# kai0511/insider

Hardware: AMD Instinct MI355X
Metric: outer-iterations/sec (masked INSIDER fit, 10000 x 50000, K=30) (higher is better)
Workload: dtype f64

## Files before the change

### insider_amd/csrc/insider_hip.hip

```cpp
#include "insider_kernels.hpp"
#include "insider_posthoc.hpp"
#include "insider_vardecomp.hpp"
#include "insider_sampdecomp.hpp"
#include "insider_levelscores.hpp"
#include "insider_factdecomp.hpp"
#include "insider_rescomp.hpp"
#include "insider_outliers.hpp"
#include "insider_neighbors.hpp"
#include "insider_coexpr.hpp"
#include "insider_coexpr_pc.hpp"
#include "insider_enrich.hpp"
#include "insider_kmeans.hpp"
#include "insider_hclust.hpp"
#include "insider_tsne.hpp"

#include <rccl/rccl.h>

#include <algorithm>
#include <chrono>
#include <cstdlib>
#include <cmath>
#include <cstdio>
#include <cstring>
#include <limits>
// ... 214 lines not shown
    std::vector<CovTables> contm;
    CovTables contm_lists;
    DevBuf<double> cont_cnt;
    bool cont_merged = false;
    std::vector<DevBuf<double>> cont_pair;
    std::shared_ptr<const HostTables> host;
    mutable std::mutex fold_mu;
    mutable std::shared_ptr<const FoldIds> folds;
    std::shared_ptr<const FoldIds> get_folds() const { std::lock_guard<std::mutex> g(fold_mu); return folds; }
    size_t bytes_shared = 0, bytes_own = 0;

    struct Block { int rows, off; };
    int blocks() const { return c + (m > 0 ? 1 : 0); }
    Block block(int b) const { return b < c ? Block{n_levels[b], lvl_off[b]} : Block{m, SLcat}; }

    DataSet() = default;
    DataSet(const DataSet &) = delete;
    DataSet &operator=(const DataSet &) = delete;
    ~DataSet() { (void)hipSetDevice(device); }
};

struct Workspace {
    static constexpr int EARLY = 3;
    int K = 0, NB = 0, KP = 0, nseg = 1;
    int gram_blocks_p = 0, gram_blocks_n = 0, sc_blocks = 0;
    DevBuf<double> Astack, R, C, RtR, CCt, Qfull, SC, stat, stat_col, gram_part, sc_part, lvl_part, eq, lvl_sum;
    DevBuf<double> fperm;
    DevBuf<double> lvl_zero;
    DevBuf<double> Qheld;
    DevBuf<double> U, Ylvl, wpart, Vlev;
    DevBuf<double> lvl_sum_all;
    DevBuf<double> gram_part2, sc_part2;
    DevBuf<double> wg_part;
    DevBuf<uint8_t> wg_pair;
    DevBuf<double> sse_train, sse_test, b2, b1, loss_buf, stage;
    size_t stage_count = 0;
    DevBuf<int> sweeps, failflag;
    DevBuf<int> sweep_key;
    DevBuf<unsigned long long> sweep_total;
    DevBuf<unsigned> pc4_ticket;
    unsigned pc4_base[2] = {0, 0};
    unsigned long long cd_code_base = 0, cd_pair_base = 0;
    DevBuf<unsigned long long> code_base_dev;
    uint8_t *order = nullptr;
    DevBuf<uint8_t> order_buf[2];
    int order_rows = 0;
    DevBuf<int> gene_perm;
    DevBuf<int> sched_cnt[2], sched_rank;
    DevBuf<uint16_t> sched_bkt;
    int sched_flip = 0;
    DevBuf<double> cd_hsave, cd_isave;
    DevBuf<uint32_t> cd_pass_slot;
    DevBuf<int> cd_pass_perm[2], cd_pass_cnt;
    DevBuf<int> perm_early[EARLY];
    bool have_early[EARLY] = {false, false, false};
    bool have_perm = false;
};

constexpr unsigned EV_SYNC = hipEventDisableTiming | hipEventDisableSystemFence;

struct Join {
    Event ev;
    bool pending = false;
    int record(hipStream_t s) { HIPCHECK(hipEventRecord(ev, s)); pending = true; return INSIDER_OK; }
    int wait(hipStream_t s)
    {
        if (pending) HIPCHECK(hipStreamWaitEvent(s, ev, 0));
        pending = false;
        return INSIDER_OK;
    }
    void drop() { pending = false; }
};

struct Streams {
    Stream stream;
    Stream side;
    Stream side2;
    Stream side3;
    Event ev_cd_done, ev_prep, ev_c_ready;
    Event ev_head;
    std::vector<Event> ev_w;
    Event ev_a_ready, ev_tab;
    Join qfull, qheld, side_done;

    int create(int n_w)
    {
        HIPCHECK(hipStreamCreate(stream.out()));
        for (Stream *s : {&side, &side2, &side3}) HIPCHECK(hipStreamCreateWithFlags(s->out(), hipStreamNonBlocking));
        for (Event *e : {&ev_prep, &ev_c_ready, &ev_head, &ev_a_ready, &qfull.ev, &qheld.ev, &ev_cd_done, &side_done.ev, &ev_tab})
            HIPCHECK(hipEventCreateWithFlags(e->out(), EV_SYNC));
        ev_w.resize(n_w);
        for (Event &e : ev_w) HIPCHECK(hipEventCreateWithFlags(e.out(), EV_SYNC));
        return INSIDER_OK;
    }
    int synchronize_sides() const
    {
        for (const Stream *s : {&side, &side2, &side3}) HIPCHECK(hipStreamSynchronize(*s));
        return INSIDER_OK;
    }
    void synchronize() const
    {
        for (const Stream *s : {&stream, &side, &side2, &side3}) if (*s) (void)hipStreamSynchronize(*s);
    }
};

struct Options {
    int max_sweeps = 1 << 24, order_mode = 0, profile = 0, verbose = 0, cd_variant = 0, force_allreduce = 0;
    int col_factored = 1;
    int row_counts = 1;
    int row_merged = 1;
    int row_gemm = 1;
    int wg_waves = 1024;
    int row_fused = 1;
    int mm_fast = 1;
    int mm_tiles = 0;
    int col_mfma4 = 1;
    int stats_own_q = 1;
    int cd_pairs = 1;
    int list_fine = 1;
    int cd_cold_iters = 3, cd_pass_first = 64, cd_pass_ratio = 4;
    double resid_stage_mb = 256.0;
    double vd_stage_kb = 48.0;
    int sd_slabs = 0;
    int ls_slabs = 0;
    double ls_part_mb = 256.0;
    int glm_slabs = 0;
    int rc_slabs = 0;
};

struct PostWs {
    DevBuf<double> Ast, U, cp, part, stats, stage, gpart, gram, cpart, gsum, L, dinv, outs;
    DevBuf<int> nz, ints, info;
    DevBuf<double> vin, vtab, vrec;
    DevBuf<double> spart, srec;
    DevBuf<double> lcand, ltab, lpart, lcnt, lout;
    DevBuf<double> fwall, fprod, fbase, frec;
    DevBuf<double> rq, rcs, rz, rpart, rin, rout;
    DevBuf<double> ocs, oz;
    DevBuf<uint32_t> obits;
    DevBuf<int> ogcnt, oscnt, orows, ocols;
    DevBuf<long long> ooffs;
};

}

struct insider_hip_handle {
    std::shared_ptr<const DataSet> ds;
    Streams st;
    Options opt;
    Workspace ws;
    PostWs post;
    FitPlan plan;
    bool w_ready = false;
    int64_t gene_offset = 0;
    int rank = 0, world = 1;
    insider_allreduce_fn allreduce = nullptr;
    void *allreduce_user = nullptr;
    ncclComm_t comm = nullptr;
    std::vector<Event> ev_col, ev_row, ev_cd, ev_test;
    double prof[12] = {0, 0, 0, 0, 0, 0, 0, 0, 0, 0, 0, 0};
    double steady_cd_ms = 0, steady_col_ms = 0;
    int cap_hits = 0, max_gene_sweeps = 0;
    int col_solver = 0, col_eval = 0, col_ridge_fallback = 0;
    int col_stats_kernel = 0, col_stats_tickets = 0, col_stats_blocks = 0;
    int col_stats_own_q = 0;
    int col_q_kernel = 0, mm_rows2_tiles = 0;
    uint64_t row_kernels = 0;
    int vd_path = 0;
    int sd_path = 0, sd_slabs = 0;
    int ls_path = 0, ls_slabs = 0;
    int glm_slabs = 0, glm_form = 0;
    int fd_path = 0;
    int ls_form = 0, fd_form = 0, rc_form = 0, cx_form = 0;
    int rc_slabs = 0;
    double rc_ms = 0.0;
    double cx_stage_mb = 0.0, cx_stage_ms = 0.0, cx_ms = 0.0, cx_pc_ms = 0.0;
    int ol_path = 0;

    ~insider_hip_handle()
    {
        if (ds) (void)hipSetDevice(ds->device);
        st.synchronize();
        if (comm) (void)ncclCommDestroy(comm);
    }
};

namespace {

enum RowKernel {
    RK_WGEMM4 = 0, RK_WGEMM5, RK_WGEMM6, RK_WGEMM7, RK_WGEMM_CHUNKS, RK_WSYRK, RK_GRAM_SIDE,
    RK_GENE_U_CNT, RK_GENE_U, RK_GENE_UC,
    RK_MERGED_SOLVE, RK_MERGED, RK_MERGED_ZERO, RK_PACK_REDUCE,
    RK_LIST_STATS4, RK_LIST_STATS, RK_LEVEL_PARTIAL, RK_LEVEL_SOLVE, RK_CONT_CD,
    RK_MM_ROWS2, RK_MM_ROWS, RK_MM_REDUCE2_2, RK_MM_REDUCE2_4, RK_MM_REDUCE
};
inline uint64_t rk_bit(RowKernel k) { return 1ull << (int)k; }
inline void row_mark(insider_hip_handle *h, RowKernel k) { h->row_kernels |= rk_bit(k); }

PlanFacts plan_facts(const insider_hip_handle *h, int K)
{
    const DataSet &d = *h->ds;
    PlanFacts f;
    const Options &o = h->opt;
    f.opt = {o.row_merged, o.col_factored, o.row_fused, o.row_gemm, o.row_counts, o.mm_fast, o.force_allreduce, o.wg_waves,
             o.list_fine, o.mm_tiles, o.col_mfma4, o.cd_variant, o.cd_pairs, o.cd_cold_iters, o.cd_pass_first, o.cd_pass_ratio, o.max_sweeps,
             o.stats_own_q};
    f.world = h->world; f.n_simd = d.n_simd;
    f.K = K; f.NB = h->ws.NB; f.KP = h->ws.KP; f.lvl_zero = (bool)h->ws.lvl_zero; f.fperm = (bool)h->ws.fperm;
    f.merged = d.merged; f.cont_merged = d.cont_merged; f.cf_pair_ok = d.cf_pair_ok; f.cf_hn = (bool)d.cf_hn; f.cf_zt = (bool)d.cf_zt; f.cf_sq = (bool)d.cf_sq;
    f.c = d.c; f.m = d.m; f.SL = d.SL; f.SLP = d.SLP; f.SLcat = d.SLcat; f.n = d.n; f.p = d.p; f.col_entries = d.col_entries; f.row_entries = d.row_entries;
    for (const CovTables &ct : d.cov) { f.L.push_back(ct.L); f.npairs.push_back(ct.npairs); }
    f.cf_c = d.cf.c; f.cf_tab_rows = d.cf.tab_rows; f.cf_nsteps = d.cf.nsteps;
    std::copy(d.cf.L, d.cf.L + CF_MAXC + 1, f.cf_L);
    std::copy(d.cf.nlater, d.cf.nlater + CF_MAXC + 1, f.cf_nlater);
    return f;
}

int ensure_workspace(insider_hip_handle *h, int K)
{
    if (K < 1 || K > INSIDER_MAX_K) return fail(INSIDER_ERR_UNSUPPORTED, "K must be in 1..63");
    if (h->ws.K == K) return INSIDER_OK;
    h->ws = Workspace();
    const DataSet &d = *h->ds;
    const hipStream_t st = h->st.stream;
    Workspace w;
    const int NB = (K + 1 + 15) / 16, KP = 16 * NB, NBLK = NB * (NB + 1) / 2, STAT = NBLK * 256;
    w.NB = NB;
    w.KP = KP;
    const int64_t avg_batches = (int64_t)(d.row_entries / (uint64_t)LIST_ALIGN / (uint64_t)std::max<int64_t>(d.n, 1));
    int nseg = (int)std::min<int64_t>(std::max<int64_t>(1, cdiv(8192, d.n)), std::max<int64_t>(1, avg_batches / 16));
    nseg = std::min(nseg, 64);
    w.nseg = nseg;
    w.gram_blocks_p = cdiv(d.p, MM_SLAB);
    w.gram_blocks_n = cdiv(d.n, MM_SLAB);
    w.sc_blocks = cdiv(d.p, MM_SLAB);
    const size_t rec = STAT + 2 * KP + 2, max_L = std::max(d.max_L, 1);
    int rc;
    if ((rc = w.Astack.alloc((size_t)(d.SL + 16) * KP))) return rc;
    HIPCHECK(hipMemset(w.Astack, 0, (size_t)(d.SL + 16) * KP * sizeof(double)));
    if ((rc = w.R.alloc((size_t)d.n * KP))) return rc;
    if ((rc = w.C.alloc((size_t)(std::max<int64_t>(d.p, d.ldp) + 4) * KP))) return rc;
    if ((rc = w.RtR.alloc((size_t)KP * KP))) return rc;
    if ((rc = w.CCt.alloc((size_t)KP * KP))) return rc;
    if ((rc = w.Qfull.alloc((size_t)d.p * KP))) return rc;
    if ((rc = w.SC.alloc((size_t)d.SL * KP))) return rc;
    if ((rc = w.stat.alloc((size_t)nseg * d.n * STAT))) return rc;
    if ((rc = w.stat_col.alloc((size_t)d.p * STAT))) return rc;
    if ((rc = w.gram_part.alloc((size_t)std::max(w.gram_blocks_p, w.gram_blocks_n) * KP * KP))) return rc;
    if ((rc = w.sc_part.alloc((size_t)w.sc_blocks * d.SL * KP))) return rc;
    if ((rc = w.lvl_part.alloc((size_t)d.max_chunks * rec))) return rc;
    if ((rc = w.lvl_sum.alloc(max_L * rec))) return rc;
    if (NB == 2 && K >= 16)
        if ((rc = w.fperm.alloc((size_t)std::max(d.n, d.p) * KP))) return rc;
    if ((rc = w.lvl_zero.alloc(max_L * rec))) return rc;
    HIPCHECK(hipMemsetAsync(w.lvl_zero, 0, max_L * rec * sizeof(double), st));
    if (d.merged) {
        size_t wg_len = 0;
        int wg_ntile = 0;
        const PlanFacts facts = plan_facts(h, K);
        for (int i = 0; i < d.c; ++i) {
            const WgPlan g = wgemm_plan(facts, i, true);
            if (g.use) {
                wg_len = std::max(wg_len, (size_t)g.nslab * (16 * g.tiles) * (16 * g.ntile));
                wg_ntile = g.ntile;
            }
        }
        if (wg_len) {
            if ((rc = w.wg_part.alloc(wg_len))) return rc;
            std::vector<uint8_t> ab((size_t)2 * 16 * wg_ntile, (uint8_t)(KP - 1));
            int idx = 0;
            for (int a = 0; a < K; ++a)
                for (int b = 0; b <= a; ++b, ++idx) {
                    ab[idx] = (uint8_t)a;
                    ab[(size_t)16 * wg_ntile + idx] = (uint8_t)b;
                }
            if ((rc = w.wg_pair.upload(ab))) return rc;
        }
        if ((rc = w.U.alloc((size_t)d.p * round_up(max_L, 2)))) return rc;
        if ((rc = w.Ylvl.alloc(max_L * KP))) return rc;
        if ((rc = w.wpart.alloc((size_t)std::max(d.max_items, 1) * STAT))) return rc;
        if ((rc = w.lvl_sum_all.alloc((size_t)std::max(d.SL, 1) * rec))) return rc;
        if ((rc = w.gram_part2.alloc((size_t)std::max(w.gram_blocks_p, w.gram_blocks_n) * KP * KP))) return rc;
        if ((rc = w.sc_part2.alloc((size_t)w.sc_blocks * d.SL * KP))) return rc;
        if ((rc = w.Vlev.alloc((size_t)d.p * d.SLP))) return rc;
        HIPCHECK(hipMemsetAsync(w.Vlev, 0, (size_t)d.p * d.SLP * sizeof(double), st));
        if ((rc = w.Qheld.alloc((size_t)d.p * KP))) return rc;
    }
    if ((rc = w.eq.alloc((size_t)d.max_L * (KP * KP + KP)))) return rc;
    for (DevBuf<double> *b : {&w.sse_train, &w.sse_test, &w.b2, &w.b1})
        if ((rc = b->alloc((size_t)d.p))) return rc;
    if ((rc = w.loss_buf.alloc(8))) return rc;
    w.stage_count = (size_t)std::max<int64_t>(std::max<int64_t>(d.p, d.n), d.SL) * KP;
    if ((rc = w.stage.alloc(w.stage_count))) return rc;
    if ((rc = w.sweeps.alloc((size_t)d.p))) return rc;
    if ((rc = w.failflag.alloc(4))) return rc;
    if ((rc = w.sweep_total.alloc(256))) return rc;
    if ((rc = w.pc4_ticket.alloc((size_t)(PC4_PARTS + 1) * 32))) return rc;
    HIPCHECK(hipMemsetAsync(w.pc4_ticket, 0, (size_t)(PC4_PARTS + 1) * 32 * sizeof(unsigned), st));
    if ((rc = w.gene_perm.alloc((size_t)d.p))) return rc;
    if ((rc = w.sched_cnt[0].alloc((size_t)SCHED_BUCKETS))) return rc;
    if ((rc = w.sched_cnt[1].alloc((size_t)SCHED_BUCKETS))) return rc;
    if ((rc = w.sched_rank.alloc((size_t)d.p))) return rc;
    if ((rc = w.sched_bkt.alloc((size_t)d.p))) return rc;
    if ((rc = w.sweep_key.alloc((size_t)d.p))) return rc;
    if ((rc = w.cd_hsave.alloc((size_t)d.p * KP))) return rc;
    if ((rc = w.cd_isave.alloc((size_t)d.p * KP))) return rc;
// ... 586 lines not shown
            HIPCHECK(hipStreamWaitEvent(h->st.side, h->st.ev_cd_done, 0));
            st = h->st.side;
        }
        if ((rc = launch_gene_order(h, h->ws.sweeps, (outer_iter < Workspace::EARLY || !h->ws.have_perm) ? 1 : 0, 0, st, fused_bucket)))
            return rc;
        h->ws.have_perm = true;
        if (early) {
            HIPCHECK(hipMemcpyAsync(h->ws.perm_early[outer_iter], h->ws.gene_perm, (size_t)h->ds->p * sizeof(int),
                                    hipMemcpyDeviceToDevice, st));
            h->ws.have_early[outer_iter] = true;
        }
        if (side) h->st.side_done.pending = true;
    }
    return INSIDER_OK;
}

int side_close(insider_hip_handle *h)
{
    return h->st.side_done.pending ? h->st.side_done.record(h->st.side) : INSIDER_OK;
}

int launch_test_sse(insider_hip_handle *h, int masked, bool timed)
{
    if (!masked) {
        HIPCHECK(hipMemsetAsync(h->ws.sse_test, 0, (size_t)h->ds->p * sizeof(double), h->st.stream));
        return INSIDER_OK;
    }
    if (h->ds->no_na) return INSIDER_OK;
    Timer t;
    int rc = t.begin(h, timed);
    if (rc) return rc;
    hipLaunchKernelGGL((k_test_sse_list<4>), dim3(cdiv(h->ds->p, 4)), dim3(256), 0, h->st.stream, (const uint32_t *)h->ds->col_ptr,
                       (const int *)h->ds->col_idx, (const double *)h->ds->col_val, (const uint8_t *)h->ds->col_flag, (int)h->ds->p,
                       (const double *)h->ws.R, (const double *)h->ws.C, h->ws.K, h->ws.KP, h->ws.sse_test);
    KCHECK();
    return t.end(h, h->ev_test);
}

void plan_call(insider_hip_handle *h, int masked, const ColCall *col = nullptr) { h->plan = build_plan(plan_facts(h, h->ws.K), masked, col); }

int launch_gene_v(insider_hip_handle *h, int q_begin, int q_end)
{
    const int N = q_end - q_begin;
    if (N <= 0) return INSIDER_OK;
    if (h->plan.v_rows2) {
        const int tiles = cdiv((int)h->ds->p, 16), tpw = h->plan.mm_tpw;
        const size_t ldsb = (size_t)4 * cdiv(h->ws.K, 16) * 64 * sizeof(double);
#define GV2_LAUNCH(NT_)                                                                                                       \
    hipLaunchKernelGGL((k_mm_rows2<NT_, true>), dim3(cdiv(cdiv(tiles, tpw), 4), cdiv(N, 16 * NT_)), dim3(256), ldsb * NT_, h->st.stream, \
                       (const double *)h->ws.C, (int64_t)h->ws.KP, (int)h->ds->p, h->ws.K,                                                \
                       (const double *)(h->ws.Astack + (size_t)q_begin * h->ws.KP), h->ws.KP, N, h->ws.Vlev + q_begin, (int64_t)h->ds->SLP, N, tpw)
        switch (mm_rows_nt(N)) {
            case 1: GV2_LAUNCH(1); break;
            case 2: GV2_LAUNCH(2); break;
            default: GV2_LAUNCH(4); break;
        }
#undef GV2_LAUNCH
        KCHECK();
        row_mark(h, RK_MM_ROWS2);
        h->mm_rows2_tiles = tpw;
        return INSIDER_OK;
    }
#define GV_LAUNCH(NT_)                                                                                                        \
    hipLaunchKernelGGL((k_mm_rows<NT_, true>), dim3(cdiv(cdiv((int)h->ds->p, 16), 4), cdiv(N, 16 * NT_)), dim3(256), 0, h->st.stream, \
                       (const double *)h->ws.C, (int64_t)h->ws.KP, (int)h->ds->p, h->ws.K,                                                \
                       (const double *)(h->ws.Astack + (size_t)q_begin * h->ws.KP), h->ws.KP, N, h->ws.Vlev + q_begin, (int64_t)h->ds->SLP, N)
    switch (mm_rows_nt(N)) {
        case 1: GV_LAUNCH(1); break;
        case 2: GV_LAUNCH(2); break;
        default: GV_LAUNCH(4); break;
    }
#undef GV_LAUNCH
    KCHECK();
    row_mark(h, RK_MM_ROWS);
    return INSIDER_OK;
}

int launch_row_stats(insider_hip_handle *h, bool timed)
{
    Timer t;
    int rc = t.begin(h, timed);
    if (rc) return rc;
    rc = launch_list_stats(h, false, h->ws.nseg, h->ws.C, h->ws.stat, nullptr, &h->row_kernels);
    if (rc) return rc;
    return t.end(h, h->ev_row);
}

int do_allreduce(insider_hip_handle *h, double *buf, int64_t count)
{
    if (!h->plan.allreduce) return INSIDER_OK;
    if (h->comm) {
        const ncclResult_t r = ncclAllReduce(buf, buf, (size_t)count, ncclDouble, ncclSum, h->comm, h->st.stream);
        if (r != ncclSuccess) return fail(INSIDER_ERR_COMM, std::string("ncclAllReduce: ") + ncclGetErrorString(r));
        return INSIDER_OK;
    }
    if (!h->allreduce) {
        if (h->world > 1) return fail(INSIDER_ERR_COMM, "world > 1 needs insider_hip_comm_init() or an all-reduce callback");
        return INSIDER_OK;
    }
    if (h->allreduce(h->allreduce_user, buf, count, (void *)h->st.stream) != 0)
        return fail(INSIDER_ERR_COMM, "all-reduce callback failed");
    return INSIDER_OK;
}

int launch_level_gram(insider_hip_handle *h, int i, hipStream_t st, double *rec, const CovTables *cont_ct = nullptr)
{
    const CovTables &ct = cont_ct ? *cont_ct : h->ds->cov[i];
    const CovTables &lists = cont_ct ? h->ds->contm_lists : ct;
    const WgPlan w = cont_ct ? WgPlan() : h->plan.wg[i];
    const int stat_len = h->plan.stat_len, plen = h->plan.plen;
    if (w.use) {
        const float *hn = h->ds->cf_hn + h->ds->cf.hn_off[h->ds->cf_pos[i]];
        const dim3 grid(cdiv(cdiv(w.ntile, 2) * w.nslab, 4), 1, w.zch);
#define WG_LAUNCH(LT_)                                                                                                     \
    hipLaunchKernelGGL((k_wgemm<LT_>), grid, dim3(256), 0, st, hn, h->ds->cf.hn_stride, w.tiles, (const double *)h->ws.C, h->ws.KP,   \
                       (int)h->ds->p, w.slab, w.nslab, (const uint8_t *)h->ws.wg_pair, w.ntile, h->ws.wg_part)
        switch (w.LT) {
            case 4: WG_LAUNCH(4); row_mark(h, RK_WGEMM4); break;
            case 5: WG_LAUNCH(5); row_mark(h, RK_WGEMM5); break;
            case 6: WG_LAUNCH(6); row_mark(h, RK_WGEMM6); break;
            default: WG_LAUNCH(7); row_mark(h, RK_WGEMM7); break;
        }
#undef WG_LAUNCH
        if (w.zch > 1) row_mark(h, RK_WGEMM_CHUNKS);
        KCHECK();
        hipLaunchKernelGGL(k_wgemm_sum, dim3(cdiv(stat_len, 256), ct.L), dim3(256), 0, st, (const double *)h->ws.wg_part, w.nslab,
                           w.tiles, w.ntile, h->ws.K, stat_len, rec, plen);
        KCHECK();
        return INSIDER_OK;
    }
    NB_DISPATCH(h->ws.NB, {
        if (ct.nitems > 0) {
            hipLaunchKernelGGL((k_wsyrk<NB_, WPB_>), dim3(cdiv(ct.nitems, WPB_)), dim3(WPB_ * 64), 0, st,
                               (const uint32_t *)lists.item_begin, (const uint32_t *)lists.item_end, ct.nitems,
                               (const int *)lists.wl_idx, (const double *)ct.wl_w, (const double *)h->ws.C, (int64_t)h->ds->p, h->ws.wpart);
            row_mark(h, RK_WSYRK);
        }
        hipLaunchKernelGGL(k_level_sum, dim3(cdiv(stat_len, 16), ct.L), dim3(256), 0, st, (const double *)h->ws.wpart,
                           (const int *)lists.lvl_item_ptr, stat_len, rec, plen);
    });
    KCHECK();
    return INSIDER_OK;
}

int launch_wsyrk_side(insider_hip_handle *h)
{
    HIPCHECK(hipEventRecord(h->st.ev_c_ready, h->st.stream));
    HIPCHECK(hipStreamWaitEvent(h->st.side2, h->st.ev_c_ready, 0));
    HIPCHECK(hipEventRecord(h->st.ev_head, h->st.side2));
    HIPCHECK(hipStreamWaitEvent(h->st.side3, h->st.ev_c_ready, 0));
    if (int rp = launch_gram(h, h->ws.C, h->ds->p, h->ws.CCt, h->st.side3, h->ws.gram_part2)) return rp;
    if (int rp = launch_mm_reduce_kp(h, h->ds->Strain, h->ds->SLP, h->ws.C, (int)h->ds->p, h->ds->SL, h->ws.sc_part2, h->ws.SC, h->st.side3)) return rp;
    HIPCHECK(hipEventRecord(h->st.ev_prep, h->st.side3));
    row_mark(h, RK_GRAM_SIDE);
    const size_t plen = h->plan.plen;
    for (int i = 0; i < h->ds->c; ++i) {
        if (int rg = launch_level_gram(h, i, h->st.side2, h->ws.lvl_sum_all + (size_t)h->ds->lvl_off[i] * plen)) return rg;
        HIPCHECK(hipEventRecord(h->st.ev_w[i], h->st.side2));
    }
    for (int k = 0; k < (h->ds->cont_merged ? h->ds->m : 0); ++k) {
        if (int rg = launch_level_gram(h, 0, h->st.side2, h->ws.lvl_sum_all + (size_t)(h->ds->SLcat + k) * plen, &h->ds->contm[k])) return rg;
        HIPCHECK(hipEventRecord(h->st.ev_w[h->ds->c + k], h->st.side2));
    }
    h->w_ready = true;
    return INSIDER_OK;
}

int row_update(insider_hip_handle *h, int i, int cont_col, int masked, double lambda1, bool rebuild_R = true)
{
    const bool cont = cont_col >= 0;
    const FitPlan &plan = h->plan;
    const bool fused_solve = !cont && plan.fused_solve;
    const CovTables &ct = cont ? h->ds->cont : h->ds->cov[i];
    const int row0 = cont ? h->ds->SLcat + cont_col : h->ds->lvl_off[i];
    LevelArgs la;
    la.stat = h->ws.stat;
    la.nseg = h->ws.nseg;
    la.n = (int)h->ds->n;
    la.K = h->ws.K;
    la.masked = masked;
    la.R = h->ws.R;
    la.lev = h->ds->lev;
    la.lvl_off = h->ds->lvl_off_d;
    la.cov = cont ? -1 : i;
    la.own_row = row0;
    la.weights = cont ? h->ds->Zc + (size_t)cont_col * h->ds->n : nullptr;
    la.chunk_begin = ct.chunk_begin;
    la.chunk_end = ct.chunk_end;
    la.members = cont ? h->ds->ident_members : h->ds->members_all + (size_t)i * h->ds->n;
    la.nchunks = ct.nchunks;
    la.Astack = h->ws.Astack;
    la.part = h->ws.lvl_part;
    LevelReduceArgs ra;
    ra.part = h->ws.lvl_sum;
    ra.L = ct.L;
    ra.K = h->ws.K;
    ra.CCt = h->ws.CCt;
    ra.SC = h->ws.SC;
    ra.sc_off = row0;
    ra.eq = h->ws.eq;
    if (cont && plan.merged) {
        const int KP = h->ws.KP;
        const CovTables &cm = h->ds->contm[cont_col];
        ColFacArgs ca = h->ds->cf;
        ca.zt = h->ds->cf_zt;
        hipLaunchKernelGGL((k_gene_uc<4>), dim3(cdiv(h->ds->p, 4)), dim3(256), 0, h->st.stream, ca, cont_col, (const double *)h->ws.Vlev, h->ds->SLP,
                           h->ws.U);
        KCHECK();
        row_mark(h, RK_GENE_UC);
        int ypart_n = 0;
        if (int rcy = launch_mm_reduce_kp(h, h->ws.U, 2, h->ws.C, (int)h->ds->p, 1, h->ws.sc_part, nullptr, nullptr, &ypart_n, &h->row_kernels))
            return rcy;
        if (h->w_ready) {
            HIPCHECK(hipStreamWaitEvent(h->st.stream, h->st.ev_w[h->ds->c + cont_col], 0));
            HIPCHECK(hipStreamWaitEvent(h->st.stream, h->st.ev_prep, 0));
        }
        double *rec = h->w_ready ? h->ws.lvl_sum_all + (size_t)row0 * plan.plen : h->ws.lvl_sum;
        if (!h->w_ready)
            if (int rg = launch_level_gram(h, 0, h->st.stream, rec, &cm)) return rg;
        NB_DISPATCH(h->ws.NB, {
            (void)WPB_;
            hipLaunchKernelGGL((k_level_merged<NB_>), dim3(1), dim3(256), 0, h->st.stream, (const double *)rec, (const double *)h->ws.sc_part,
                               ypart_n, (const double *)cm.paircnt, h->ds->SL, (const double *)h->ws.Astack, (const int *)h->ds->one_count,
                               (const double *)h->ws.CCt, (const double *)(h->ws.SC + (size_t)row0 * KP), 1, h->ws.K, lambda1, 0, h->ws.eq,
                               h->ws.Astack + (size_t)row0 * KP, h->ws.failflag, (const double *)(h->ds->cont_cnt + cont_col));
        });
        row_mark(h, RK_MERGED);
    } else if (!cont && plan.merged) {
        const int L = ct.L, LP = (int)round_up(L, 2), KP = h->ws.KP;
        if (plan.u_cnt[i]) {
            const size_t gu_lds = (size_t)4 * (h->ds->SL + LP + GU_BATCH * WAVE) * sizeof(double);
            ColFacArgs ca = h->ds->cf;
            ca.cnt = h->ds->cf_cnt;
            ca.zt = h->ds->m > 0 ? h->ds->cf_zt : nullptr;
            hipLaunchKernelGGL((k_gene_u_cnt<4>), dim3(cdiv(h->ds->p, 4)), dim3(256), gu_lds, h->st.stream, ca, h->ds->cf_pos[i], LP,
                               (const double *)h->ws.Vlev, h->ds->SLP, h->ds->SL, h->ws.U);
            row_mark(h, RK_GENE_U_CNT);
        } else {
            if (h->ds->m > 0) return fail(INSIDER_ERR_UNSUPPORTED, "merged row update with continuous covariates needs the pair-count form");
            hipLaunchKernelGGL((k_gene_u<4>), dim3(cdiv(h->ds->p, 4)), dim3(256), (size_t)4 * (h->ds->SLcat + GU_TILE) * sizeof(double),
                               h->st.stream, (const uint32_t *)ct.grp, (const uint16_t *)ct.slev,
                               (size_t)h->ds->col_entries + LIST_BLOCK, h->ds->c - 1, L, LP, (const double *)h->ws.Vlev, h->ds->SLP, (int)h->ds->p,
                               h->ds->SLcat, h->ws.U);
            row_mark(h, RK_GENE_U);
        }
        KCHECK();
        int ypart_n = 0;
        if (int rcy = launch_mm_reduce_kp(h, h->ws.U, LP, h->ws.C, (int)h->ds->p, L, h->ws.sc_part, plan.row_fused ? nullptr : h->ws.Ylvl, nullptr,
                                          &ypart_n, &h->row_kernels))
            return rcy;
        if (!plan.row_fused) ypart_n = 0;
        if (h->w_ready) {
            HIPCHECK(hipStreamWaitEvent(h->st.stream, h->st.ev_w[i], 0));
            HIPCHECK(hipStreamWaitEvent(h->st.stream, h->st.ev_prep, 0));
        }
        if (!h->w_ready)
            if (int rg = launch_level_gram(h, i, h->st.stream, h->ws.lvl_sum)) return rg;
        double *rec = h->w_ready ? h->ws.lvl_sum_all + (size_t)row0 * plan.plen : h->ws.lvl_sum;
        NB_DISPATCH(h->ws.NB, {
            (void)WPB_;
            if (plan.row_fused) {
                hipLaunchKernelGGL((k_level_merged<NB_>), dim3(L), dim3(256), 0, h->st.stream, (const double *)rec,
                                   (const double *)(ypart_n ? h->ws.sc_part : h->ws.Ylvl), ypart_n, (const double *)ct.paircnt, h->ds->SL, (const double *)h->ws.Astack,
                                   (const int *)(h->ds->lvl_count_all + h->ds->lvl_off[i]), (const double *)h->ws.CCt,
                                   (const double *)(h->ws.SC + (size_t)row0 * KP), L, h->ws.K, lambda1, fused_solve ? 1 : 0, h->ws.eq,
                                   h->ws.Astack + (size_t)row0 * KP, h->ws.failflag);
                row_mark(h, fused_solve ? RK_MERGED_SOLVE : RK_MERGED);
            } else {
                hipLaunchKernelGGL(k_level_pack, dim3(L), dim3(256), 0, h->st.stream, (const double *)h->ws.Ylvl,
                                   (const double *)ct.paircnt, h->ds->SL, (const double *)h->ws.Astack,
                                   (const int *)(h->ds->lvl_count_all + h->ds->lvl_off[i]), L, h->ws.K, KP, plan.stat_len, rec);
                ra.part = rec;
                hipLaunchKernelGGL((k_level_reduce<NB_>), dim3(L), dim3(64), 0, h->st.stream, ra);
                row_mark(h, RK_PACK_REDUCE);
            }
        });
    } else if (!cont && plan.unmasked_fused) {
        const int L = ct.L, KP = h->ws.KP;
        NB_DISPATCH(h->ws.NB, {
            (void)WPB_;
            hipLaunchKernelGGL((k_level_merged<NB_>), dim3(L), dim3(256), 0, h->st.stream, (const double *)h->ws.lvl_zero,
                               (const double *)h->ws.lvl_zero, 0, (const double *)ct.paircnt, h->ds->SL, (const double *)h->ws.Astack,
                               (const int *)(h->ds->lvl_count_all + h->ds->lvl_off[i]), (const double *)h->ws.CCt,
                               (const double *)(h->ws.SC + (size_t)row0 * KP), L, h->ws.K, lambda1, fused_solve ? 1 : 0, h->ws.eq,
                               h->ws.Astack + (size_t)row0 * KP, h->ws.failflag);
        });
        row_mark(h, fused_solve ? RK_MERGED_SOLVE : RK_MERGED);
        row_mark(h, RK_MERGED_ZERO);
    } else {
        NB_DISPATCH(h->ws.NB, {
            (void)WPB_;
            hipLaunchKernelGGL((k_level_partial<NB_>), dim3(ct.nchunks), dim3(64), 0, h->st.stream, la);
            hipLaunchKernelGGL(k_level_sum, dim3(cdiv(plan.plen, 16), ct.L), dim3(256), 0, h->st.stream,
                               (const double *)h->ws.lvl_part, (const int *)ct.lvl_chunk_ptr, plan.plen, h->ws.lvl_sum, plan.plen);
            hipLaunchKernelGGL((k_level_reduce<NB_>), dim3(ct.L), dim3(64), 0, h->st.stream, ra);
        });
        row_mark(h, RK_LEVEL_PARTIAL);
    }
    KCHECK();
    if (fused_solve) return rebuild_R ? launch_build_R(h) : INSIDER_OK;
    int rc = do_allreduce(h, h->ws.eq, (int64_t)ct.L * (h->ws.KP * h->ws.KP + h->ws.KP));
    if (rc) return rc;
    if (cont && masked) {
        NB_DISPATCH(h->ws.NB, {
            (void)WPB_;
            hipLaunchKernelGGL((k_cont_cd<NB_>), dim3(1), dim3(64), 0, h->st.stream, (const double *)h->ws.eq, h->ws.K, lambda1,
                               h->ws.Astack + (size_t)row0 * h->ws.KP);
        });
        row_mark(h, RK_CONT_CD);
    } else {
        NB_DISPATCH(h->ws.NB, {
            (void)WPB_;
            hipLaunchKernelGGL((k_level_solve<NB_>), dim3(ct.L), dim3(64), 0, h->st.stream, (const double *)h->ws.eq,
                               (const int *)(cont ? h->ds->one_count : h->ds->lvl_count_all + h->ds->lvl_off[i]), ct.L, h->ws.K, lambda1,
                               h->ws.Astack + (size_t)row0 * h->ws.KP, h->ws.failflag);
        });
        row_mark(h, RK_LEVEL_SOLVE);
    }
    KCHECK();
    return rebuild_R ? launch_build_R(h) : INSIDER_OK;
}

struct LossOut {
    double sum_residual, train_rmse, test_rmse, row_reg_half, col_reg_half, l1_reg, loss;
};

int loss_checkpoint(insider_hip_handle *h, int tuning, double lambda1, double lambda2, double alpha, LossOut *o)
{
    hipLaunchKernelGGL(k_loss_reduce, dim3(1), dim3(256), 0, h->st.stream, h->ws.sse_train, h->ws.sse_test, h->ws.b2, h->ws.b1,
                       (int)h->ds->p, h->ws.Astack, h->ds->SL, h->ws.K, h->ws.KP, h->ws.loss_buf);
    KCHECK();
    double cnt[2] = {tuning == 1 ? h->ds->cnt_train : (double)h->ds->n * (double)h->ds->p, h->ds->cnt_test};
    HIPCHECK(hipMemcpyAsync(h->ws.loss_buf + 4, cnt, 2 * sizeof(double), hipMemcpyHostToDevice, h->st.stream));
    int rc = do_allreduce(h, h->ws.loss_buf, 6);
    if (rc) return rc;
    double v[8];
    HIPCHECK(hipMemcpyAsync(v, h->ws.loss_buf, 8 * sizeof(double), hipMemcpyDeviceToHost, h->st.stream));
    HIPCHECK(hipStreamSynchronize(h->st.stream));
    o->sum_residual = v[0];
    o->train_rmse = std::sqrt(v[0] / v[4]);
    o->test_rmse = (tuning == 1 && v[5] > 0) ? std::sqrt(v[1] / v[5]) : std::numeric_limits<double>::quiet_NaN();
    const double nfA = std::sqrt(v[6]), nfC = std::sqrt(v[2]);
    o->row_reg_half = lambda1 * nfA * nfA / 2;
    o->col_reg_half = lambda2 * (1 - alpha) * nfC * nfC / 2;
    o->l1_reg = lambda2 * alpha * v[3];
    o->loss = o->sum_residual / 2 + o->row_reg_half + o->col_reg_half + o->l1_reg;
    return INSIDER_OK;
}

int check_fail_flag(insider_hip_handle *h)
{
    int f = 0;
    HIPCHECK(hipMemcpyAsync(&f, h->ws.failflag, sizeof(int), hipMemcpyDeviceToHost, h->st.stream));
    HIPCHECK(hipStreamSynchronize(h->st.stream));
    if (f) {
        HIPCHECK(hipMemsetAsync(h->ws.failflag, 0, sizeof(int), h->st.stream));
        return fail(INSIDER_ERR_SOLVE, "a ridge normal-equation system was not positive definite");
    }
    return INSIDER_OK;
}

int read_cap_hits(insider_hip_handle *h)
{
    int v[2] = {0, 0};
    HIPCHECK(hipMemcpyAsync(v, h->ws.failflag + 2, sizeof(v), hipMemcpyDeviceToHost, h->st.stream));
    HIPCHECK(hipStreamSynchronize(h->st.stream));
    h->cap_hits = v[0];
    h->max_gene_sweeps = v[1];
    return INSIDER_OK;
}

void clear_events(insider_hip_handle *h)
{
    for (auto *v : {&h->ev_col, &h->ev_row, &h->ev_cd, &h->ev_test}) v->clear();
}

int upload_factors(insider_hip_handle *h, double *const *A, const double *C, int K)
{
    const DataSet &d = *h->ds;
    const int KP = h->ws.KP;
    const hipStream_t st = h->st.stream;
    for (int b = 0; b < d.blocks(); ++b) {
        const DataSet::Block blk = d.block(b);
        HIPCHECK(hipMemcpyAsync(h->ws.stage, A[b], (size_t)blk.rows * K * sizeof(double), hipMemcpyHostToDevice, st));
        hipLaunchKernelGGL(k_pack_A, dim3(cdiv(blk.rows * KP, 256)), dim3(256), 0, st, (const double *)h->ws.stage, blk.rows, K, KP,
                           h->ws.Astack + (size_t)blk.off * KP);
        KCHECK();
        HIPCHECK(hipStreamSynchronize(st));
    }
    if (!C) return INSIDER_OK;
    HIPCHECK(hipMemcpyAsync(h->ws.stage, C, (size_t)d.p * K * sizeof(double), hipMemcpyHostToDevice, st));
    hipLaunchKernelGGL(k_pack_rows, dim3(cdiv(d.p * KP, 256)), dim3(256), 0, st, (const double *)h->ws.stage, d.p, K, KP, h->ws.C);
    KCHECK();
    return INSIDER_OK;
}

int download_factors(insider_hip_handle *h, double *const *A, double *C, int K)
{
    const DataSet &d = *h->ds;
    const int KP = h->ws.KP;
    const hipStream_t st = h->st.stream;
    for (int b = 0; A && b < d.blocks(); ++b) {
        const DataSet::Block blk = d.block(b);
        hipLaunchKernelGGL(k_unpack_A, dim3(cdiv(blk.rows * K, 256)), dim3(256), 0, st,
                           (const double *)(h->ws.Astack + (size_t)blk.off * KP), blk.rows, K, KP, h->ws.stage);
        KCHECK();
        HIPCHECK(hipMemcpyAsync(A[b], h->ws.stage, (size_t)blk.rows * K * sizeof(double), hipMemcpyDeviceToHost, st));
        HIPCHECK(hipStreamSynchronize(st));
// ... 3358 lines not shown
```

### insider_amd/csrc/insider_row_merged.hpp

```cpp
#pragma once

namespace insider {

__global__ void __launch_bounds__(256) k_group_count(const uint32_t *__restrict__ col_ptr, const int *__restrict__ col_idx,
                                                     const int *__restrict__ lev , int L, int p,
                                                     uint32_t *__restrict__ grp )
{
    extern __shared__ int s_hist[];
    const int w = threadIdx.x >> 6, lane = threadIdx.x & 63;
    const int j = blockIdx.x * 4 + w;
    if (j >= p) return;
    int *hist = s_hist + w * L;
    for (int l = lane; l < L; l += WAVE) hist[l] = 0;
    wave_sync();
    for (uint32_t e = col_ptr[j] + lane; e < col_ptr[j + 1]; e += WAVE) {
        const int r = col_idx[e];
        if (r != LIST_PAD) atomicAdd(&hist[lev[r]], 1);
    }
    wave_sync();
    const int seg = (L + WAVE - 1) / WAVE, l0 = lane * seg, l1 = l0 + seg < L ? l0 + seg : L;
    int run = 0;
    for (int l = l0; l < l1; ++l) run += hist[l];
    int incl = run;
    for (int o = 1; o < WAVE; o <<= 1) {
// ... 183 lines not shown
        ld(0, ia, xa);
        ld(1, ib, xb);
        for (int blk = 0; blk < nblk; ++blk) {
            int *li = s_li[w][blk & 1];
            double *lx = s_lw[w][blk & 1];
#pragma unroll
            for (int t = 0; t < EPL; ++t) { li[t * WAVE + lane] = ia[t]; lx[t * WAVE + lane] = xa[t]; }
#pragma unroll
            for (int t = 0; t < EPL; ++t) { ia[t] = ib[t]; xa[t] = xb[t]; }
            ld(blk + 2, ib, xb);
            wave_sync();
            const int left = nbt - blk * (LIST_BLOCK / SYRK_BATCH);
            const int nbatch = __builtin_amdgcn_readfirstlane(left < LIST_BLOCK / SYRK_BATCH ? left : LIST_BLOCK / SYRK_BATCH);
            double a0[SYRK_GB][NB], w0[SYRK_GB][NB], a1[SYRK_GB][NB], w1[SYRK_GB][NB];
            wsyrk_load<NB>(li, lx, 0, rsrc, a0, w0, lane);
            for (int b = 0; b < nbatch; b += 2) {
                wsyrk_load<NB>(li, lx, b + 1, rsrc, a1, w1, lane);
                wsyrk_mfma<NB>(a0, w0, acc);
                wsyrk_load<NB>(li, lx, b + 2 < nbatch ? b + 2 : nbatch - 1, rsrc, a0, w0, lane);
                wsyrk_mfma<NB>(a1, w1, acc);
            }
        }
    }
    double *out = stat + (size_t)item * Geo<NB>::STAT;
    const int sub = lane >> 4, c16 = lane & 15;
#pragma unroll
    for (int b = 0; b < NBLK; ++b)
#pragma unroll
        for (int r = 0; r < 4; ++r) out[b * 256 + (sub + 4 * r) * 16 + c16] = acc[b][r];
}

template <int LT>
__global__ void __launch_bounds__(256)
k_wgemm(const float *__restrict__ hn, int hn_stride, int lt_total, const double *__restrict__ C, int KP, int p, int slab, int nslab,
        const uint8_t *__restrict__ pair_ab , int ntile, double *__restrict__ part )
{
    const int w = __builtin_amdgcn_readfirstlane(threadIdx.x >> 6), lane = threadIdx.x & 63;
    const int per = (ntile + 1) >> 1;
    const int W = blockIdx.x * 4 + w;
    if (W >= per * nslab) return;
    const int slab_id = W / per;
    const int T0 = (W - slab_id * per) * 2;
    const int lt0 = blockIdx.z * LT;
    const int g4 = lane >> 4, c16 = lane & 15;
    const int j_begin = slab_id * slab, j_end = j_begin + slab < p ? j_begin + slab : p;
    unsigned off_a[2], off_b[2];
#pragma unroll
    for (int t = 0; t < 2; ++t) {
        const int T = T0 + t < ntile ? T0 + t : ntile - 1;
        off_a[t] = 8u * (unsigned)(g4 * KP + pair_ab[16 * T + c16]);
        off_b[t] = 8u * (unsigned)(g4 * KP + pair_ab[16 * ntile + 16 * T + c16]);
    }
    const unsigned off_n = 4u * (unsigned)(g4 * hn_stride + (c16 & 3) * 4 + (c16 >> 2));
    d4 acc[LT][2];
#pragma unroll
    for (int l = 0; l < LT; ++l)
#pragma unroll
        for (int t = 0; t < 2; ++t) acc[l][t] = d4{0.0, 0.0, 0.0, 0.0};
    struct Ops { float n[LT]; double ca[2], cb[2]; };
    auto fetch = [&](int j0, Ops &o) {
        const char *hb = reinterpret_cast<const char *>(hn + (size_t)j0 * hn_stride + 16 * lt0);
        const char *cb = reinterpret_cast<const char *>(C + (size_t)j0 * KP);
#pragma unroll
        for (int l = 0; l < LT; ++l) o.n[l] = *reinterpret_cast<const float *>(hb + off_n + 64 * l);
#pragma unroll
        for (int t = 0; t < 2; ++t) {
            o.ca[t] = *reinterpret_cast<const double *>(cb + off_a[t]);
            o.cb[t] = *reinterpret_cast<const double *>(cb + off_b[t]);
        }
    };
    auto compute = [&](const Ops &o) {
        double b[2];
#pragma unroll
        for (int t = 0; t < 2; ++t) b[t] = o.ca[t] * o.cb[t];
#pragma unroll
        for (int l = 0; l < LT; ++l) {
            const double a = (double)o.n[l];
#pragma unroll
            for (int t = 0; t < 2; ++t) acc[l][t] = __builtin_amdgcn_mfma_f64_16x16x4f64(a, b[t], acc[l][t], 0, 0, 0);
        }
    };
    Ops o0, o1, o2;
    if (j_begin < j_end) fetch(j_begin, o0);
    if (j_begin + 4 < j_end) fetch(j_begin + 4, o1);
    for (int j0 = j_begin; j0 < j_end; j0 += 12) {
        if (j0 + 8 < j_end) fetch(j0 + 8, o2);
        compute(o0);
        if (j0 + 4 < j_end) {
            if (j0 + 12 < j_end) fetch(j0 + 12, o0);
            compute(o1);
            if (j0 + 8 < j_end) {
                if (j0 + 16 < j_end) fetch(j0 + 16, o1);
                compute(o2);
            }
        }
    }
    double *out = part + (size_t)slab_id * (16 * lt_total) * (16 * ntile);
#pragma unroll
    for (int l = 0; l < LT; ++l)
        if (lt0 + l < lt_total) {
#pragma unroll
            for (int t = 0; t < 2; ++t)
                if (T0 + t < ntile) {
#pragma unroll
                    for (int r = 0; r < 4; ++r)
                        out[(size_t)(16 * (lt0 + l) + g4 + 4 * r) * (16 * ntile) + 16 * (T0 + t) + c16] = acc[l][t][r];
                }
        }
}

__global__ void __launch_bounds__(256) k_wgemm_sum(const double *__restrict__ part, int nslab, int lt_total, int ntile, int K,
                                                   int stat_len, double *__restrict__ rec, int plen)
{
    const int e = blockIdx.x * 256 + threadIdx.x, l = blockIdx.y;
    if (e >= stat_len) return;
    int blk = e >> 8, bi = 0;
    while ((bi + 1) * (bi + 2) / 2 <= blk) ++bi;
    const int bj = blk - bi * (bi + 1) / 2;
    const int a = 16 * bi + ((e >> 4) & 15), b = 16 * bj + (e & 15);
    double s = 0.0;
    if (a < K && b < K) {
        const int hi = a > b ? a : b, lo = a > b ? b : a;
        const size_t stride = (size_t)(16 * lt_total) * (16 * ntile);
        const double *src = part + (size_t)l * (16 * ntile) + (hi * (hi + 1) / 2 + lo);
#pragma unroll 8
        for (int sl = 0; sl < nslab; ++sl) s += src[(size_t)sl * stride];
        s *= 2.0;
    }
    rec[(size_t)l * plen + e] = s;
}

__global__ void __launch_bounds__(256) k_level_pack(const double *__restrict__ Y ,
                                                    const double *__restrict__ paircnt , int SL,
                                                    const double *__restrict__ Astack, const int *__restrict__ lvl_count,
                                                    int L, int K, int KP, int stat_len, double *__restrict__ rec)
{
    __shared__ double red[4][64];
    const int l = blockIdx.x, k = threadIdx.x & 63, g = threadIdx.x >> 6;
    if (l >= L) return;
    double ss = 0.0;
    if (k < K)
        for (int q = g; q < SL; q += 4) ss = fma(paircnt[(size_t)l * SL + q], Astack[(size_t)q * KP + k], ss);
    red[g][k] = ss;
    __syncthreads();
    if (g != 0) return;
    double *out = rec + (size_t)l * (stat_len + 2 * KP + 2) + stat_len;
    if (k < KP) {
        out[k] = k < K ? Y[(size_t)l * KP + k] : 0.0;
        out[KP + k] = ((red[0][k] + red[1][k]) + red[2][k]) + red[3][k];
    }
    if (k == 0) { out[2 * KP] = (double)lvl_count[l]; out[2 * KP + 1] = 0.0; }
}

template <int NB>
__global__ void __launch_bounds__(256) k_level_merged(const double *__restrict__ rec ,
                                                      const double *__restrict__ Y , int ypart_n,
                                                      const double *__restrict__ paircnt , int SL,
                                                      const double *__restrict__ Astack, const int *__restrict__ lvl_count,
                                                      const double *__restrict__ CCt, const double *__restrict__ SC ,
                                                      int L, int K, double lambda, int do_solve, double *__restrict__ eq,
                                                      double *__restrict__ Arows , int *__restrict__ fail,
                                                      const double *__restrict__ cnt_real = nullptr )
{
    constexpr int KP = Geo<NB>::KP, NBLK = Geo<NB>::NBLK, STAT = Geo<NB>::STAT;
    __shared__ double red[4][64];
    __shared__ double s_H[KP * KP];
    __shared__ double s_A[NB <= 2 ? KP * KP : 1];
    __shared__ double s_s[KP];
    __shared__ double s_y[16][KP];
    const int l = blockIdx.x, lane = threadIdx.x & 63, g = threadIdx.x >> 6;
    if (l >= L) return;
    if (ypart_n > 0) {
        const size_t len = (size_t)L * KP;
        for (int c = threadIdx.x; c < 16 * KP; c += 256) {
            const int m = c / KP, o = c % KP;
            double sm = 0.0;
#pragma unroll 8
            for (int b = m; b < ypart_n; b += 16) sm += Y[(size_t)b * len + (size_t)l * KP + o];
            s_y[m][o] = sm;
        }
    }
    double ss = 0.0;
    if (lane < K)
        for (int q = g; q < SL; q += 4) ss = fma(paircnt[(size_t)l * SL + q], Astack[(size_t)q * KP + lane], ss);
    red[g][lane] = ss;
    __syncthreads();
    if (g != 0) return;
    const bool valid = lane < K;
    const int sub = lane >> 4, c16 = lane & 15;
    const double cnt = cnt_real ? cnt_real[l] : (double)lvl_count[l];
    double v = 0.0;
    if (valid) {
        if (ypart_n > 0) {
#pragma unroll
            for (int m = 0; m < 16; ++m) v += s_y[m][lane];
        } else {
            v = Y[(size_t)l * KP + lane];
        }
    }
    const double ssum = ((red[0][lane] + red[1][lane]) + red[2][lane]) + red[3][lane];
    const double *src = rec + (size_t)l * (STAT + 2 * KP + 2);
    d4 h[NBLK];
#pragma unroll
    for (int b = 0; b < NBLK; ++b)
#pragma unroll
        for (int q = 0; q < 4; ++q) h[b][q] = src[b * 256 + (sub + 4 * q) * 16 + c16];
    acc_to_lds<NB>(h, s_H, lane);
    if (lane < KP) s_s[lane] = ssum;
    wave_sync();
    double *eql = eq + (size_t)l * (KP * KP + KP);
    for (int i = lane; i < KP * KP; i += WAVE) {
        const int x = i / KP, y = i % KP;
        const double e = (x < K && y < K) ? cnt * CCt[i] - s_H[i] : 0.0;
        eql[i] = e;
        if constexpr (NB <= 2) s_A[i] = e;
    }
    double yv = 0.0;
    if (lane < KP) {
        if (valid) {
            yv = SC[(size_t)l * KP + lane] + v;
            for (int b = 0; b < K; ++b) yv -= CCt[b * KP + lane] * s_s[b];
        }
        eql[KP * KP + lane] = yv;
    }
    if constexpr (NB <= 2) {
        if (!do_solve || cnt_real || lvl_count[l] == 0) return;
        wave_sync();
        double b = lane < KP ? yv : 0.0;
        double row[KP];
#pragma unroll
        for (int c = 0; c < KP; ++c) row[c] = lane < KP ? s_A[c * KP + lane] : 0.0;
#pragma unroll
        for (int c = 0; c < KP; ++c) row[c] += (c == lane && lane < K) ? lambda : 0.0;
        if (!gj_solve_regs<KP>(row, K, b, lane)) {
            wave_sync();
            if (lane < K) s_A[lane * KP + lane] += lambda;
            b = lane < KP ? yv : 0.0;
            wave_sync();
            if (!lu_solve_lds(s_A, KP, K, b, lane)) { if (lane == 0) *fail = 1; return; }
        }
        if (lane < K) Arows[(size_t)l * KP + lane] = b;
    }
}

}
```

Measured before the change: 705.9.

## Prefetch and batch loads in k_level_merged, skip redundant prep-event waits

Reworks k_level_merged so all global loads (rec accumulator, SC, level counts, CCt) are issued at kernel start. The Y partial reduction and the paircnt·Astack dot product are restructured into unrolled, double-buffered batches of independent loads, and CCt is staged in LDS. The goal is more memory-level parallelism and less exposed latency in this single-level-per-block kernel. Host side, the ev_prep wait is now issued once per side launch instead of before every row update. This raises register and LDS use, which could lower occupancy.

```diff
diff --git a/insider_amd/csrc/insider_hip.hip b/insider_amd/csrc/insider_hip.hip
--- a/insider_amd/csrc/insider_hip.hip
+++ b/insider_amd/csrc/insider_hip.hip
@@ -390,6 +390,7 @@
     PostWs post;
     FitPlan plan;
     bool w_ready = false;
+    bool prep_joined = false;
     int64_t gene_offset = 0;
     int rank = 0, world = 1;
     insider_allreduce_fn allreduce = nullptr;
@@ -1282,6 +1283,7 @@
     if (int rp = launch_gram(h, h->ws.C, h->ds->p, h->ws.CCt, h->st.side3, h->ws.gram_part2)) return rp;
     if (int rp = launch_mm_reduce_kp(h, h->ds->Strain, h->ds->SLP, h->ws.C, (int)h->ds->p, h->ds->SL, h->ws.sc_part2, h->ws.SC, h->st.side3)) return rp;
     HIPCHECK(hipEventRecord(h->st.ev_prep, h->st.side3));
+    h->prep_joined = false;
     row_mark(h, RK_GRAM_SIDE);
     const size_t plen = h->plan.plen;
     for (int i = 0; i < h->ds->c; ++i) {
@@ -1293,6 +1295,14 @@
         HIPCHECK(hipEventRecord(h->st.ev_w[h->ds->c + k], h->st.side2));
     }
     h->w_ready = true;
+    return INSIDER_OK;
+}
+
+int join_side(insider_hip_handle *h, int w)
+{
+    HIPCHECK(hipStreamWaitEvent(h->st.stream, h->st.ev_w[w], 0));
+    if (!h->prep_joined) HIPCHECK(hipStreamWaitEvent(h->st.stream, h->st.ev_prep, 0));
+    h->prep_joined = true;
     return INSIDER_OK;
 }
 
@@ -1341,10 +1351,8 @@
         int ypart_n = 0;
         if (int rcy = launch_mm_reduce_kp(h, h->ws.U, 2, h->ws.C, (int)h->ds->p, 1, h->ws.sc_part, nullptr, nullptr, &ypart_n, &h->row_kernels))
             return rcy;
-        if (h->w_ready) {
-            HIPCHECK(hipStreamWaitEvent(h->st.stream, h->st.ev_w[h->ds->c + cont_col], 0));
-            HIPCHECK(hipStreamWaitEvent(h->st.stream, h->st.ev_prep, 0));
-        }
+        if (h->w_ready)
+            if (int rj = join_side(h, h->ds->c + cont_col)) return rj;
         double *rec = h->w_ready ? h->ws.lvl_sum_all + (size_t)row0 * plan.plen : h->ws.lvl_sum;
         if (!h->w_ready)
             if (int rg = launch_level_gram(h, 0, h->st.stream, rec, &cm)) return rg;
@@ -1380,10 +1388,8 @@
                                           &ypart_n, &h->row_kernels))
             return rcy;
         if (!plan.row_fused) ypart_n = 0;
-        if (h->w_ready) {
-            HIPCHECK(hipStreamWaitEvent(h->st.stream, h->st.ev_w[i], 0));
-            HIPCHECK(hipStreamWaitEvent(h->st.stream, h->st.ev_prep, 0));
-        }
+        if (h->w_ready)
+            if (int rj = join_side(h, i)) return rj;
         if (!h->w_ready)
             if (int rg = launch_level_gram(h, i, h->st.stream, h->ws.lvl_sum)) return rg;
         double *rec = h->w_ready ? h->ws.lvl_sum_all + (size_t)row0 * plan.plen : h->ws.lvl_sum;
diff --git a/insider_amd/csrc/insider_row_merged.hpp b/insider_amd/csrc/insider_row_merged.hpp
--- a/insider_amd/csrc/insider_row_merged.hpp
+++ b/insider_amd/csrc/insider_row_merged.hpp
@@ -359,6 +359,8 @@
     if (k == 0) { out[2 * KP] = (double)lvl_count[l]; out[2 * KP + 1] = 0.0; }
 }
 
+constexpr int LM_YCH = 32;
+constexpr int LM_SCH = 16;
 template <int NB>
 __global__ void __launch_bounds__(256) k_level_merged(const double *__restrict__ rec ,
                                                       const double *__restrict__ Y , int ypart_n,
@@ -370,32 +372,93 @@
                                                       const double *__restrict__ cnt_real = nullptr )
 {
     constexpr int KP = Geo<NB>::KP, NBLK = Geo<NB>::NBLK, STAT = Geo<NB>::STAT;
+    constexpr bool STAGE = NB <= 2;
+    constexpr int CPT = STAGE ? KP * KP / 256 : 1;
     __shared__ double red[4][64];
     __shared__ double s_H[KP * KP];
     __shared__ double s_A[NB <= 2 ? KP * KP : 1];
+    __shared__ double s_C[STAGE ? KP * KP : 1];
     __shared__ double s_s[KP];
     __shared__ double s_y[16][KP];
     const int l = blockIdx.x, lane = threadIdx.x & 63, g = threadIdx.x >> 6;
     if (l >= L) return;
+    const bool valid = lane < K;
+    double ccr[CPT];
+    if constexpr (STAGE) {
+#pragma unroll
+        for (int t = 0; t < CPT; ++t) ccr[t] = CCt[threadIdx.x + 256 * t];
+    }
+    const int sub = lane >> 4, c16 = lane & 15;
+    d4 h[NBLK];
+    double scv = 0.0, cnt = 0.0;
+    int nl = 0;
+    if (g == 0) {
+        const double *src = rec + (size_t)l * (STAT + 2 * KP + 2);
+#pragma unroll
+        for (int b = 0; b < NBLK; ++b)
+#pragma unroll
+            for (int q = 0; q < 4; ++q) h[b][q] = src[b * 256 + (sub + 4 * q) * 16 + c16];
+        if (valid) scv = SC[(size_t)l * KP + lane];
+        nl = lvl_count[l];
+        cnt = cnt_real ? cnt_real[l] : (double)nl;
+    }
+    const double *pc = paircnt + (size_t)l * SL, *as = Astack + (valid ? lane : 0);
+    auto ss_fetch = [&](int q0, double (&a)[LM_SCH], double (&b)[LM_SCH]) {
+#pragma unroll
+        for (int i = 0; i < LM_SCH; ++i) {
+            const int q = q0 + 4 * i < SL ? q0 + 4 * i : 0;
+            a[i] = pc[q];
+            b[i] = as[(size_t)q * KP];
+        }
+    };
+    double pa0[LM_SCH], pb0[LM_SCH], pa1[LM_SCH], pb1[LM_SCH];
+    ss_fetch(g, pa0, pb0);
     if (ypart_n > 0) {
         const size_t len = (size_t)L * KP;
-        for (int c = threadIdx.x; c < 16 * KP; c += 256) {
-            const int m = c / KP, o = c % KP;
-            double sm = 0.0;
-#pragma unroll 8
-            for (int b = m; b < ypart_n; b += 16) sm += Y[(size_t)b * len + (size_t)l * KP + o];
-            s_y[m][o] = sm;
+        for (int c0 = threadIdx.x; c0 < 16 * KP; c0 += 512) {
+            const int c1 = c0 + 256 < 16 * KP ? c0 + 256 : c0;
+            const int m0 = c0 / KP, m1 = c1 / KP;
+            const uint32_t lo0 = (uint32_t)(l * KP + c0 % KP), lo1 = (uint32_t)(l * KP + c1 % KP);
+            const uint32_t of0 = (uint32_t)(m0 * len) + lo0, of1 = (uint32_t)(m1 * len) + lo1;
+            double sm0 = 0.0, sm1 = 0.0;
+            for (int b0 = 0; b0 < ypart_n; b0 += 16 * LM_YCH) {
+                double r0[LM_YCH], r1[LM_YCH];
+#pragma unroll
+                for (int i = 0; i < LM_YCH; ++i) {
+                    const int bu = b0 + 16 * i;
+                    const double *slab = Y + (bu < ypart_n ? (size_t)bu * len : 0);
+                    r0[i] = slab[bu + m0 < ypart_n ? of0 : lo0];
+                    r1[i] = slab[bu + m1 < ypart_n ? of1 : lo1];
+                }
+#pragma unroll
+                for (int i = 0; i < LM_YCH; ++i) sm0 = b0 + 16 * i + m0 < ypart_n ? sm0 + r0[i] : sm0;
+#pragma unroll
+                for (int i = 0; i < LM_YCH; ++i) sm1 = b0 + 16 * i + m1 < ypart_n ? sm1 + r1[i] : sm1;
+            }
+            s_y[m0][c0 % KP] = sm0;
+            s_y[m1][c1 % KP] = sm1;
         }
     }
     double ss = 0.0;
-    if (lane < K)
-        for (int q = g; q < SL; q += 4) ss = fma(paircnt[(size_t)l * SL + q], Astack[(size_t)q * KP + lane], ss);
+    auto ss_chain = [&](int q0, const double (&a)[LM_SCH], const double (&b)[LM_SCH]) {
+#pragma unroll
+        for (int i = 0; i < LM_SCH; ++i) ss = q0 + 4 * i < SL ? fma(a[i], b[i], ss) : ss;
+    };
+    for (int q0 = g; q0 < SL; q0 += 8 * LM_SCH) {
+        ss_fetch(q0 + 4 * LM_SCH, pa1, pb1);
+        ss_chain(q0, pa0, pb0);
+        ss_fetch(q0 + 8 * LM_SCH, pa0, pb0);
+        ss_chain(q0 + 4 * LM_SCH, pa1, pb1);
+    }
+    if (!valid) ss = 0.0;
+    if constexpr (STAGE) {
+#pragma unroll
+        for (int t = 0; t < CPT; ++t) s_C[threadIdx.x + 256 * t] = ccr[t];
+    }
     red[g][lane] = ss;
     __syncthreads();
     if (g != 0) return;
-    const bool valid = lane < K;
-    const int sub = lane >> 4, c16 = lane & 15;
-    const double cnt = cnt_real ? cnt_real[l] : (double)lvl_count[l];
+    const double *cc = STAGE ? s_C : CCt;
     double v = 0.0;
     if (valid) {
         if (ypart_n > 0) {
@@ -406,32 +469,26 @@
         }
     }
     const double ssum = ((red[0][lane] + red[1][lane]) + red[2][lane]) + red[3][lane];
-    const double *src = rec + (size_t)l * (STAT + 2 * KP + 2);
-    d4 h[NBLK];
-#pragma unroll
-    for (int b = 0; b < NBLK; ++b)
-#pragma unroll
-        for (int q = 0; q < 4; ++q) h[b][q] = src[b * 256 + (sub + 4 * q) * 16 + c16];
     acc_to_lds<NB>(h, s_H, lane);
     if (lane < KP) s_s[lane] = ssum;
     wave_sync();
     double *eql = eq + (size_t)l * (KP * KP + KP);
     for (int i = lane; i < KP * KP; i += WAVE) {
         const int x = i / KP, y = i % KP;
-        const double e = (x < K && y < K) ? cnt * CCt[i] - s_H[i] : 0.0;
+        const double e = (x < K && y < K) ? cnt * cc[i] - s_H[i] : 0.0;
         eql[i] = e;
         if constexpr (NB <= 2) s_A[i] = e;
     }
     double yv = 0.0;
     if (lane < KP) {
         if (valid) {
-            yv = SC[(size_t)l * KP + lane] + v;
-            for (int b = 0; b < K; ++b) yv -= CCt[b * KP + lane] * s_s[b];
+            yv = scv + v;
+            for (int b = 0; b < K; ++b) yv -= cc[b * KP + lane] * s_s[b];
         }
         eql[KP * KP + lane] = yv;
     }
     if constexpr (NB <= 2) {
-        if (!do_solve || cnt_real || lvl_count[l] == 0) return;
+        if (!do_solve || cnt_real || nl == 0) return;
         wave_sync();
         double b = lane < KP ? yv : 0.0;
         double row[KP];
```

Measured after the change: 717.1 (median of 6 runs). +1.6%, better.
